# li-guihai/slam-dynamic

Measured on AMD Instinct MI355X. Metric: tracking frames/sec (extract+match+dynamic-cull), KITTI 1241x376, higher is better.
Workload: dtype u8+f32; 1 GPU; KITTI stereo 1241x376 colour pairs, 2000 feat/image: YOLOv3 (640x480, f32 as the reference's cv::dnn, synthetic weights) on the left image -> boxes -> TrackStereo = cvtColor + 2x ORB extract + stereo match + boxTrack + firstSeparate + TrackHomo (SearchByProjection vs the queued frame > 0.2 s back, H/F fit) + Separate + UpdateFrame + SearchByProjection vs the last frame (BASELINE configs[2]); spec ; lanes_per_gpu=256, images_per_frame=2, detector_arithmetic=f32 operands, f32 accumulation (v_mfma_f32_32x32x2_f32), max_detector_boxes_in_a_frame=29

## Files before the change

slam-dynamic_amd/csrc/k_yolo32.h:

```cpp
#pragma once
#include "k_yolo.h"

typedef float sd_f4 __attribute__((ext_vector_type(4)));

struct SdConvArgsF {
    const float* in; const float* wgt; const float* bias; const float* res; float* out;
    const float* zero;
    int N, H, W, cin, cinStride;
    int Ho, Wo, cout, outStride, resStride;
    int ksize, stride, pad, leaky;
    int pair;
    int tilesX, tilesY, groupY;
};

template <int BK, int WM, int MT, int NW>
__global__ void __launch_bounds__(64 * NW, NW == 8 ? 1 : (WM == 2 && BK == 16 ? 3 : 2)) k_conv_f32(SdConvArgsF A)
{
    constexpr int NT = 64 * NW;
    constexpr int WN = NW / WM, BM = 32 * MT * WM, BN = 64 * WN;
    constexpr int LD = BK + 4;
    constexpr int CPR = BK / 4;
    constexpr int XC = (BN * CPR + NT - 1) / NT;
    constexpr int WC = (BM * CPR + NT - 1) / NT;
    constexpr int STAGE = (BM + BN) * LD;
    constexpr int NCH = BK / 8;
    extern __shared__ __align__(16) float smemf[];
    const int tid = threadIdx.x, lane = tid & 63, wv = tid >> 6, r32 = lane & 31, h = lane >> 5;
    const int wm = wv % WM, wn = wv / WM;
    const int perXcd = (A.tilesX + 7) >> 3;
    const int slot = blockIdx.x >> 3, perGroup = perXcd * A.groupY;
    const int grp = slot / perGroup, r = slot - grp * perGroup;
    const int tx = (blockIdx.x & 7) * perXcd + r / A.groupY, ty = grp * A.groupY + r % A.groupY;
    if (tx >= A.tilesX) return;
    const int pix0 = tx * BN, co0 = ty * BM;
    const int npix = A.N * A.Ho * A.Wo;
    int pyi[XC], pxi[XC];
    size_t pbase[XC];
    bool pok[XC];
#pragma unroll
    for (int i = 0; i < XC; i++) {
        const int chunk = tid + NT * i;
        const int p = pix0 + chunk / CPR;
        pok[i] = chunk < BN * CPR && p < npix;
        const int pp = pok[i] ? p : 0;
        const int n = pp / (A.Ho * A.Wo), r = pp - n * (A.Ho * A.Wo);
        const int yo = r / A.Wo, xo = r - yo * A.Wo;
        pyi[i] = yo * A.stride - A.pad; pxi[i] = xo * A.stride - A.pad;
        pbase[i] = (size_t)n * A.H * A.W;
    }
    const int taps = A.ksize * A.ksize;
    const bool pair = BK == 8 && A.pair;
    const int ksteps = pair ? (taps + 1) / 2 : taps * (A.cin / BK);
    const int wrow = pair ? 8 * ksteps : taps * A.cin;
    sd_f16v acc[MT][2];
#pragma unroll
    for (int m = 0; m < MT; m++)
#pragma unroll
        for (int n = 0; n < 2; n++)
#pragma unroll
            for (int r = 0; r < 16; r++) acc[m][n][r] = 0.f;
    constexpr bool DEEP = !(WM == 1 && MT == 2);
    constexpr int NSET = DEEP ? 2 : 1;
    sd_f4 xr[NSET][XC], wr[NSET][WC];
    const float* wptr[WC];
    const float* xptr[XC];
    int winc[WC], xinc[XC];
#pragma unroll
    for (int i = 0; i < WC; i++) {
        const int chunk = tid + NT * i;
        const bool on = chunk < BM * CPR;
        wptr[i] = on ? A.wgt + (size_t)(co0 + chunk / CPR) * wrow + 4 * (chunk % CPR) : A.zero;
        winc[i] = on ? BK : 0;
    }
    int c0 = 0, kh = 0, kw = 0, ps = 0;
    auto retap = [&]() {
#pragma unroll
        for (int i = 0; i < XC; i++) {
            const int chunk = tid + NT * i;
            int dy = kh, dx = kw, coff = 4 * (chunk % CPR);
            bool tapok = true;
            if (BK == 8 && pair) {
                const int tap = 2 * ps + (chunk % CPR);
                dy = tap / A.ksize; dx = tap - dy * A.ksize; coff = 0;
                tapok = tap < taps;
            }
            const int yi = pyi[i] + dy, xi = pxi[i] + dx;
            const bool ok = pok[i] && tapok && yi >= 0 && yi < A.H && xi >= 0 && xi < A.W;
            const float* p = A.in + ((ptrdiff_t)pbase[i] + (ptrdiff_t)yi * A.W + xi) * A.cinStride + coff;
            xptr[i] = ok ? p : A.zero;
            xinc[i] = ok && !pair ? BK : 0;
        }
    };
    retap();
    auto fetch = [&](const int set) {
#pragma unroll
        for (int i = 0; i < WC; i++) { wr[set][i] = *(const sd_f4*)wptr[i]; wptr[i] += winc[i]; }
#pragma unroll
        for (int i = 0; i < XC; i++) { xr[set][i] = *(const sd_f4*)xptr[i]; xptr[i] += xinc[i]; }
        if (BK == 8 && pair) { ps++; retap(); return; }
        c0 += BK;
        if (c0 == A.cin) { c0 = 0; kw++; if (kw == A.ksize) { kw = 0; kh++; } retap(); }
    };
    auto store = [&](int buf, const int set) {
        float* sW = smemf + buf * STAGE;
        float* sX = sW + BM * LD;
#pragma unroll
        for (int i = 0; i < WC; i++) { const int chunk = tid + NT * i; if ((WC * NT == BM * CPR) || chunk < BM * CPR) *(sd_f4*)(sW + (chunk / CPR) * LD + 4 * (chunk % CPR)) = wr[set][i]; }
#pragma unroll
        for (int i = 0; i < XC; i++) { const int chunk = tid + NT * i; if ((XC * NT == BN * CPR) || chunk < BN * CPR) *(sd_f4*)(sX + (chunk / CPR) * LD + 4 * (chunk % CPR)) = xr[set][i]; }
    };
    const int aoff = (32 * MT * wm + r32) * LD + 4 * h, boff = BM * LD + (64 * wn + r32) * LD + 4 * h;
    sd_f4 fa[2][MT], fb[2][2];
    auto frags = [&](int buf, int kc, int slot) {
        const float* base = smemf + buf * STAGE;
#pragma unroll
        for (int m = 0; m < MT; m++) fa[slot][m] = *(const sd_f4*)(base + aoff + 32 * m * LD + 8 * kc);
#pragma unroll
        for (int n = 0; n < 2; n++) fb[slot][n] = *(const sd_f4*)(base + boff + 32 * n * LD + 8 * kc);
    };
    auto mfmas = [&](int slot) {
#pragma unroll
        for (int j = 0; j < 4; j++)
#pragma unroll
            for (int m = 0; m < MT; m++)
#pragma unroll
                for (int n = 0; n < 2; n++)
                    acc[m][n] = __builtin_amdgcn_mfma_f32_32x32x2f32(fa[slot][m][j], fb[slot][n][j], acc[m][n], 0, 0, 0);
    };
    const int myslot = NW == 8 ? (NCH >= 4 ? 2 * (wv >> 2) : (NCH == 2 ? (wv >> 2) : 0)) : 0;
    float* const sBias = smemf + 2 * STAGE;
    sd_f4 bq = sd_f4{0.f, 0.f, 0.f, 0.f};
    if (tid < BM / 4 && co0 + 4 * tid < A.cout) bq = *(const sd_f4*)(A.bias + co0 + 4 * tid);
    fetch(0);
    store(0, 0);
    if (tid < BM / 4) *(sd_f4*)(sBias + 4 * tid) = bq;
    if (ksteps > 1) fetch(NSET - 1);
    if (DEEP && ksteps > 2) fetch(0);
    __syncthreads();
    auto step = [&](const int ks, const int par) {
        const int cur = par;
        frags(cur, 0, 0);
#pragma unroll
        for (int kc = 0; kc < NCH; kc++) {
            if (kc + 1 < NCH) frags(cur, kc + 1, (kc + 1) & 1);
            mfmas(kc & 1);
            if (kc == myslot) {
                if (ks + 1 < ksteps) store(cur ^ 1, DEEP ? par ^ 1 : 0);
                if (ks + 1 + NSET < ksteps) fetch(DEEP ? par ^ 1 : 0);
            }
        }
        __builtin_amdgcn_sched_barrier(0);
        __syncthreads();
        __builtin_amdgcn_sched_barrier(0);
    };
    int ks = 0;
    for (; ks + 1 < ksteps; ks += 2) { step(ks, 0); step(ks + 1, 1); }
    if (ks < ksteps) step(ks, 0);
    if constexpr (WM == 1) {
        constexpr int TWD = 32 * MT, TLD = TWD + 4;
        constexpr int PPI = 64 / (TWD / 4);
        static_assert(NW * 32 * TLD <= 2 * STAGE, "the transpose tiles of the epilogue must fit the staging buffers");
        float* T = smemf + wv * 32 * TLD;
        const int piece = lane % (TWD / 4), prow = lane / (TWD / 4);
        const int cob = co0 + TWD * wm + 4 * piece;
        const sd_f4 bias4 = *(const sd_f4*)(sBias + TWD * wm + 4 * piece);
        __syncthreads();
        auto tail = [&](const bool res, const bool inside) {
            sd_f4 rr[2][32 / PPI];
            if (res) {
#pragma unroll
                for (int n = 0; n < 2; n++)
#pragma unroll
                    for (int it = 0; it < 32 / PPI; it++) {
                        const int p = pix0 + 64 * wn + 32 * n + PPI * it + prow;
                        rr[n][it] = sd_f4{0.f, 0.f, 0.f, 0.f};
                        if (inside || (p < npix && cob < A.cout)) rr[n][it] = *(const sd_f4*)(A.res + (size_t)p * A.resStride + cob);
                    }
                __builtin_amdgcn_s_waitcnt(0x0F70);
            }
#pragma unroll
            for (int n = 0; n < 2; n++) {
#pragma unroll
                for (int m = 0; m < MT; m++)
#pragma unroll
                    for (int g = 0; g < 4; g++)
                        *(sd_f4*)(T + r32 * TLD + 32 * m + 8 * g + 4 * h) = sd_f4{acc[m][n][4 * g], acc[m][n][4 * g + 1], acc[m][n][4 * g + 2], acc[m][n][4 * g + 3]};
                __builtin_amdgcn_fence(__ATOMIC_RELEASE, "wavefront"); __builtin_amdgcn_wave_barrier(); __builtin_amdgcn_fence(__ATOMIC_ACQUIRE, "wavefront");
                const int pb = pix0 + 64 * wn + 32 * n;
#pragma unroll
                for (int it = 0; it < 32 / PPI; it++) {
                    const int pl = PPI * it + prow, p = pb + pl;
                    if (!inside && (p >= npix || cob >= A.cout)) continue;
                    const sd_f4 a = *(const sd_f4*)(T + pl * TLD + 4 * piece);
                    sd_f4 v;
#pragma unroll
                    for (int e = 0; e < 4; e++) {
                        float x = a[e] + bias4[e];
                        if (A.leaky) x = x > 0.f ? x : 0.1f * x;
                        v[e] = x + (res ? rr[n][it][e] : 0.f);
                    }
                    float* dst = A.out + (size_t)p * A.outStride + cob;
                    if (inside || cob + 3 < A.cout) *(sd_f4*)dst = v;
                    else for (int e = 0; e < 4 && cob + e < A.cout; e++) dst[e] = v[e];
                }
                __builtin_amdgcn_fence(__ATOMIC_RELEASE, "wavefront"); __builtin_amdgcn_wave_barrier(); __builtin_amdgcn_fence(__ATOMIC_ACQUIRE, "wavefront");
            }
        };
        const bool inside = pix0 + BN <= npix && co0 + BM <= A.cout;
        if (A.res) { if (inside) tail(true, true); else tail(true, false); }
        else { if (inside) tail(false, true); else tail(false, false); }
    } else {
        auto tail = [&](const bool res, const bool inside) {
            sd_f4 rr[2][MT][4];
            if (res) {
#pragma unroll
                for (int n = 0; n < 2; n++) {
                    const int p = pix0 + 64 * wn + 32 * n + r32;
#pragma unroll
                    for (int m = 0; m < MT; m++)
#pragma unroll
                        for (int g = 0; g < 4; g++) {
                            const int co = co0 + 32 * MT * wm + 32 * m + 8 * g + 4 * h;
                            rr[n][m][g] = sd_f4{0.f, 0.f, 0.f, 0.f};
                            if (inside || (p < npix && co < A.cout)) rr[n][m][g] = *(const sd_f4*)(A.res + (size_t)p * A.resStride + co);
                        }
                }
                __builtin_amdgcn_s_waitcnt(0x0F70);
            }
#pragma unroll
            for (int n = 0; n < 2; n++) {
                const int p = pix0 + 64 * wn + 32 * n + r32;
                if (!inside && p >= npix) continue;
#pragma unroll
                for (int m = 0; m < MT; m++)
#pragma unroll
                    for (int g = 0; g < 4; g++) {
                        const int cl = 32 * MT * wm + 32 * m + 8 * g + 4 * h, co = co0 + cl;
                        if (!inside && co >= A.cout) continue;
                        const sd_f4 b4 = *(const sd_f4*)(sBias + cl);
                        sd_f4 v;
#pragma unroll
                        for (int e = 0; e < 4; e++) {
                            float x = acc[m][n][4 * g + e] + b4[e];
                            if (A.leaky) x = x > 0.f ? x : 0.1f * x;
                            v[e] = x + (res ? rr[n][m][g][e] : 0.f);
                        }
                        float* dst = A.out + (size_t)p * A.outStride + co;
                        if (inside || co + 3 < A.cout) *(sd_f4*)dst = v;
                        else for (int e = 0; e < 4 && co + e < A.cout; e++) dst[e] = v[e];
                    }
            }
        };
        const bool inside = pix0 + BN <= npix && co0 + BM <= A.cout;
        if (A.res) { if (inside) tail(true, true); else tail(true, false); }
        else { if (inside) tail(false, true); else tail(false, false); }
    }
}
#define SD_F32_LDS(BK, WM, MT, NW) (2 * (32 * (MT) * (WM) + 64 * ((NW) / (WM))) * ((BK) + 4) * 4 + 32 * (MT) * (WM) * 4)

__global__ void __launch_bounds__(256) k_blob_from_image_f32(const uint8_t* __restrict__ src, int sw, int sh, size_t sstride, size_t spitch,
                                                             const short4* __restrict__ ct, const short4* __restrict__ rt,
                                                             float* __restrict__ dst, int dw, int dh, int swapRB)
{
    const int img = blockIdx.z;
    const int x = blockIdx.x * 64 + threadIdx.x, y = blockIdx.y * 4 + threadIdx.y;
    if (x >= dw || y >= dh) return;
    const short4 ce = ct[x], re = rt[y];
    const int sx = ce.x, sx1 = min(sx + 1, sw - 1);
    const int r0 = min(max((int)re.x, 0), sh - 1), r1 = min(max((int)re.x + 1, 0), sh - 1);
    const uint8_t* S0 = src + (size_t)img * spitch + (size_t)r0 * sstride;
    const uint8_t* S1 = src + (size_t)img * spitch + (size_t)r1 * sstride;
    uint32_t a0, a1, b0, b1;
    if (sx1 == sx + 1) {
        typedef uint32_t __attribute__((aligned(1))) u32u; typedef uint16_t __attribute__((aligned(1))) u16u;
        a0 = *(const u32u*)(S0 + 3 * sx); b0 = *(const u16u*)(S0 + 3 * sx + 4);
        a1 = *(const u32u*)(S1 + 3 * sx); b1 = *(const u16u*)(S1 + 3 * sx + 4);
    } else {
        a0 = (uint32_t)S0[3 * sx] | ((uint32_t)S0[3 * sx + 1] << 8) | ((uint32_t)S0[3 * sx + 2] << 16) | ((uint32_t)S0[3 * sx1] << 24);
        b0 = (uint32_t)S0[3 * sx1 + 1] | ((uint32_t)S0[3 * sx1 + 2] << 8);
        a1 = (uint32_t)S1[3 * sx] | ((uint32_t)S1[3 * sx + 1] << 8) | ((uint32_t)S1[3 * sx + 2] << 16) | ((uint32_t)S1[3 * sx1] << 24);
        b1 = (uint32_t)S1[3 * sx1 + 1] | ((uint32_t)S1[3 * sx1 + 2] << 8);
    }
    const int p0[6] = {(int)(a0 & 255), (int)((a0 >> 8) & 255), (int)((a0 >> 16) & 255), (int)(a0 >> 24), (int)(b0 & 255), (int)((b0 >> 8) & 255)};
    const int p1[6] = {(int)(a1 & 255), (int)((a1 >> 8) & 255), (int)((a1 >> 16) & 255), (int)(a1 >> 24), (int)(b1 & 255), (int)((b1 >> 8) & 255)};
    float ch[3];
#pragma unroll
    for (int c = 0; c < 3; c++) {
        const int h0 = p0[c] * ce.y + p0[3 + c] * ce.z;
        const int h1 = p1[c] * ce.y + p1[3 + c] * ce.z;
        const int v = ((((int)re.y * (h0 >> 4)) >> 16) + (((int)re.z * (h1 >> 4)) >> 16) + 2) >> 2;
        ch[c] = (float)(v & 255) * (float)(1 / 255.0);
    }
    float* o = dst + ((size_t)img * dh * dw + (size_t)y * dw + x) * 4;
    *(sd_f4*)o = sd_f4{swapRB ? ch[2] : ch[0], ch[1], swapRB ? ch[0] : ch[2], 0.f};
}


__global__ void __launch_bounds__(256) k_upsample_into_f32(const float* __restrict__ a, int C1, int aStride, int h, int w, float* __restrict__ out, int Ct, int N)
{
    const int q = C1 / 4, H2 = 2 * h, W2 = 2 * w;
    const size_t total = (size_t)N * H2 * W2 * q;
    for (size_t i = (size_t)blockIdx.x * 256 + threadIdx.x; i < total; i += (size_t)gridDim.x * 256) {
        const int c4 = (int)(i % q);
        const size_t p = i / q;
        const int x = (int)(p % W2);
        const size_t r = p / W2;
        const int y = (int)(r % H2), n = (int)(r / H2);
        *(sd_f4*)(out + p * Ct + 4 * c4) = *(const sd_f4*)(a + (((size_t)n * h + (y >> 1)) * w + (x >> 1)) * aStride + 4 * c4);
    }
}
```

slam-dynamic_amd/csrc/sd_yolo_api.hip:

```cpp
#include <hip/hip_runtime.h>
#include <cstdio>
#include <cstdlib>
#include <cstring>
#include <cstddef>
#include <cmath>
#include <string>
#include <memory>
#include <vector>
#include "sd_common.h"
#include "sd_yolo.h"

template <typename T>
static void yolo_decode(const sd_yolo* y, const sd_yolo_layer& l, const sd_yolo::Rt& r, int n, float conf_threshold, int rowBase, hipStream_t s)
{
    const float* an = y->anchors;
    const int rows = n * r.H * r.W * 3;
    hipLaunchKernelGGL(HIP_KERNEL_NAME(k_region_decode<T>), dim3((rows + 255) / 256), dim3(256), 0, s, r.as<const T>(), r.outC, r.H, r.W, n, an[2 * l.mask[0]],
                       an[2 * l.mask[0] + 1], an[2 * l.mask[1]], an[2 * l.mask[1] + 1], an[2 * l.mask[2]], an[2 * l.mask[2] + 1],
                       y->netW, y->netH, conf_threshold, rowBase, y->d_dets, y->d_ndet, y->detCap, n == 1 ? y->d_raw : nullptr);
}

extern "C" {

int sd_yolo_v3_layers(sd_yolo_layer* layers, int cap, int* n, float anchors[18])
{
    if (!n) return SD_ERR_INVALID;
    std::vector<sd_yolo_layer> L;
    yolo_v3_layers(L);
    *n = (int)L.size();
    if (anchors) memcpy(anchors, kYoloV3Anchors, sizeof(kYoloV3Anchors));
    if (layers) {
        if (cap < (int)L.size()) return set_err(SD_ERR_CAPACITY, "layer buffer too small");
        memcpy(layers, L.data(), L.size() * sizeof(sd_yolo_layer));
    }
    return SD_OK;
}

static const void* const kYoloKernelFn[SD_YK_COUNT] = {
#define X(id, block, ...) (const void*)__VA_ARGS__,
    SD_YOLO_KERNELS(X)
#undef X
};

static int yolo_kernel_lds(int k, int width)
{
    switch (k) {
    case SD_YK_GLDS_8_1: case SD_YK_GLDS_8_3: return 3 * (512 * 64 + SD_G3_WBYTES);
    case SD_YK_GLDS_4_1: case SD_YK_GLDS_4_3: return 3 * (256 * 64 + SD_G3_WBYTES);
    case SD_YK_G3_80: return SD_G3_LDS(80);
    case SD_YK_G3_160: return SD_G3_LDS(160);
    case SD_YK_F32_8_1_1_8: return SD_F32_LDS(8, 1, 1, 8);
    case SD_YK_F32_16_1_1_4: return SD_F32_LDS(16, 1, 1, 4);
    case SD_YK_F32_16_1_2_4: return SD_F32_LDS(16, 1, 2, 4);
    case SD_YK_F32_16_2_2_4: return SD_F32_LDS(16, 2, 2, 4);
    case SD_YK_WINO_16_2: return SD_WINO_LDS(16, 2);
    case SD_YK_B3_1: return SD_B3_LDS(1);
    case SD_YK_B3_2: return SD_B3_LDS(2);
    case SD_YK_B3F_3: case SD_YK_B3F_4: case SD_YK_B3F_5: case SD_YK_B3F_8: return SD_B3F_LDS(width, 128);
    case SD_YK_B3C_5: case SD_YK_B3C_6: return SD_B3C_LDS(width);
    default: return 0;
    }
}

static int yolo_launch(const SdYoloLaunch& K, void** args, hipStream_t s)
{
    (void)hipLaunchKernel(kYoloKernelFn[K.kernel], dim3(K.gridX, K.gridY), dim3(K.block), args, (size_t)yolo_kernel_lds(K.kernel, K.width), s);
    LAUNCH_CHECK(kYoloKernelInfo[K.kernel].name);
    return SD_OK;
}

static int yolo_raise_lds_limits(const sd_yolo* y)
{
    for (int k = y->f32 ? SD_YK_F32_FIRST : 0; k < (y->f32 ? SD_YK_COUNT : SD_YK_F32_FIRST); k++)
        HIPCHK(sd_raise_lds_limit(kYoloKernelFn[k], yolo_kernel_lds(k, k >= SD_YK_B3C_5 ? SD_B3C_MAXW : SD_B3F_MAXW)));
    HIPCHK(sd_raise_lds_limit((const void*)k_yolo_nms, SD_NMS_LDS));
    return SD_OK;
}

int sd_yolo_create(sd_yolo** out, const sd_yolo_layer* layers, int n_layers, const float anchors[18], int classes, int net_w,
                   int net_h, int max_batch)
{
    return sd_yolo_create_prec(out, layers, n_layers, anchors, classes, net_w, net_h, max_batch, SD_YOLO_F16);
}

int sd_yolo_create_prec(sd_yolo** out, const sd_yolo_layer* layers, int n_layers, const float anchors[18], int classes, int net_w,
                        int net_h, int max_batch, int precision)
{
// ... 286 lines not shown
int sd_yolo_mfma_flops(const sd_yolo* y, double* flops_per_image)
{
    if (!y || !flops_per_image) return SD_ERR_INVALID;
    *flops_per_image = y->mfmaFlops;
    return SD_OK;
}

int sd_yolo_forward_device(sd_yolo* y, const uint8_t* d_bgr, int width, int height, size_t stride, size_t image_pitch, int n,
                           float conf_threshold, void* stream_)
{
    if (!y || !d_bgr || width < 2 || height < 2 || n < 1 || n > y->maxBatch || width > 8192 || height > 8192) return set_err(SD_ERR_INVALID, "bad forward arguments");
    if (!y->weightsLoaded) return set_err(SD_ERR_STATE, "detector weights not loaded");
    hipStream_t s = stream_ ? (hipStream_t)stream_ : y->stream;
    if (y->tabW != width || y->tabH != height) {
        std::vector<int16_t> ct, rt;
        yolo_resize_tables(width, height, y->netW, y->netH, ct, rt);
        HIPCHK(hipMemcpy(y->d_ct, ct.data(), ct.size() * 2, hipMemcpyHostToDevice));
        HIPCHK(hipMemcpy(y->d_rt, rt.data(), rt.size() * 2, hipMemcpyHostToDevice));
        y->tabW = width; y->tabH = height;
    }
    const bool f32 = y->f32, ov = y->overlap;
    hipStream_t sb = ov ? y->sPre : s, sd = ov ? y->sPost : s;
    if (ov && y->haveL0) HIPCHK(hipStreamWaitEvent(sb, y->evL0, 0));
    {
        dim3 blk(64, 4), grd((y->netW + 63) / 64, (y->netH + 3) / 4, n);
        if (f32) hipLaunchKernelGGL(k_blob_from_image_f32, grd, blk, 0, sb, d_bgr, width, height, stride, image_pitch, y->d_ct, y->d_rt, y->d_blob8, y->netW, y->netH, 1);
        else hipLaunchKernelGGL(k_blob_from_image, grd, blk, 0, sb, d_bgr, width, height, stride, image_pitch, y->d_ct, y->d_rt, y->d_blob4, y->netW, y->netH, 1);
    }
    LAUNCH_CHECK(f32 ? "k_blob_from_image_f32" : "k_blob_from_image");
    if (ov) {
        HIPCHK(hipEventRecord(y->evBlob, sb));
        HIPCHK(hipStreamWaitEvent(s, y->evBlob, 0));
    }
    bool cleared = !f32;
    if (cleared) HIPCHK(hipMemsetAsync(y->d_ndet, 0, (size_t)n * 4, s));
    int head = 0;
    bool headGuard = ov && y->haveDecoded;
    const void* cur = f32 ? (const void*)y->d_blob8.get() : (const void*)y->d_blob4.get();
    int H = y->netH, W = y->netW, Cs = f32 ? 4 : 32;
    int rowBase = 0;
    for (size_t i = 0; i < y->L.size(); i++) {
        const sd_yolo_layer& l = y->L[i];
        const sd_yolo::Rt& r = y->R[i];
        if (l.type == SD_YOLO_CONV) {
            if (headGuard && i + 1 < y->L.size() && y->L[i + 1].type == SD_YOLO_YOLO) { HIPCHK(hipStreamWaitEvent(s, y->evDecoded, 0)); headGuard = false; }
            const SdYoloLaunch K = yolo_plan_launch(l, r, i == 0, n);
            const void* bias = y->d_bias + r.bOff;
            const void* res = nullptr; int resStride = 0;
            if (i + 1 < y->L.size() && y->L[i + 1].type == SD_YOLO_SHORTCUT && y->R[i + 1].alias) {
                const sd_yolo::Rt& rf = y->R[yolo_resolve((int)i + 1, y->L[i + 1].from[0])];
                res = rf.out; resStride = rf.outC;
            }
            int rc;
            if (K.kernel == SD_YK_CONV_FIRST) {
                const _Float16* blob = y->d_blob4; const _Float16* wgt = y->d_wgt + r.wOff; _Float16* out = r.as<_Float16>();
                int Ho = r.H, Wo = r.W, cout = l.filters, outStride = r.outC, leaky = l.leaky;
                void* args[] = {&blob, &wgt, &bias, &out, &n, &Ho, &Wo, &cout, &outStride, &leaky};
                rc = yolo_launch(K, args, s);
            } else if (r.cls == SD_YC_F16) {
                SdConvArgs A;
                A.zero = y->d_zero; A.in = (const _Float16*)cur; A.wgt = y->d_wgt + r.wOff; A.bias = (const float*)bias; A.res = (const _Float16*)res; A.out = r.as<_Float16>();
                A.N = n; A.H = H; A.W = W; A.cin = r.cinPad; A.cinStride = Cs;
                A.Ho = r.H; A.Wo = r.W; A.cout = l.filters; A.coutPad = r.coutPad; A.outStride = r.outC; A.outOff = 0; A.resStride = resStride;
                A.ksize = l.size; A.stride = l.stride; A.pad = l.size / 2; A.leaky = l.leaky;
                void* args[] = {&A};
                rc = yolo_launch(K, args, s);
            } else if (r.cls == SD_YC_WINO) {
                SdWinoArgs A;
                A.V = y->d_V; A.U = y->d_wgtW + r.wOffW; A.bias = (const float*)bias; A.res = (const float*)res; A.out = r.as<float>(); A.zero = (const float*)y->d_zero.get();
                A.N = n; A.H = r.H; A.W = r.W; A.th = (r.H + 1) / 2; A.tw = (r.W + 1) / 2;
                A.cin = r.cinPad; A.cout = l.filters; A.outStride = r.outC; A.resStride = resStride; A.leaky = l.leaky;
                A.tilesX = K.tilesX; A.tilesY = K.tilesY; A.groupY = K.groupY;
                hipLaunchKernelGGL(k_wino_input, dim3(K.inputGrid), dim3(256), 0, s, (const float*)cur, n, H, W, r.cinPad, Cs, A.th, A.tw, y->d_V);
                LAUNCH_CHECK("k_wino_input");
                void* args[] = {&A};
                rc = yolo_launch(K, args, s);
            } else {
                SdConvArgsF A;
                A.in = (const float*)cur; A.wgt = y->d_wgt32 + r.wOff; A.bias = (const float*)bias; A.res = (const float*)res; A.out = r.as<float>(); A.zero = (const float*)y->d_zero.get();
                A.N = n; A.H = H; A.W = W; A.cin = i == 0 ? 8 : r.cinPad; A.cinStride = Cs; A.pair = i == 0 ? 1 : 0;
                A.Ho = r.H; A.Wo = r.W; A.cout = l.filters; A.outStride = r.outC; A.resStride = resStride;
                A.ksize = l.size; A.stride = l.stride; A.pad = l.size / 2; A.leaky = l.leaky;
                A.tilesX = K.tilesX; A.tilesY = K.tilesY; A.groupY = K.groupY;
                const uint4* wq = y->d_wgtB + r.wOffB;
                void* args[] = {&A, &wq};
                rc = yolo_launch(K, args, s);
            }
            if (rc != SD_OK) return rc;
        } else if (l.type == SD_YOLO_SHORTCUT) {
            if (!r.alias) return set_err(SD_ERR_UNSUPPORTED, "unfused [shortcut] is not implemented");
        } else if (l.type == SD_YOLO_ROUTE && l.nfrom == 2) {
            const int fa = yolo_resolve((int)i, l.from[0]), fb = yolo_resolve((int)i, l.from[1]);
            const int src = yolo_resolve(fa, -1);
            const sd_yolo::Rt& ra = y->R[src]; const sd_yolo::Rt& rb = y->R[fb];
            if (f32 && r.alias) {
                const size_t quads = (size_t)n * r.H * r.W * (ra.C / 4);
                hipLaunchKernelGGL(k_upsample_into_f32, dim3((unsigned)std::min<size_t>((quads + 255) / 256, 4096)), dim3(256), 0, s, ra.as<const float>(), ra.C, ra.outC, ra.H, ra.W,
                                   r.as<float>(), r.C, n);
                LAUNCH_CHECK("k_upsample_into_f32");
            } else {
                const int hc = f32 ? 2 : 1, piece = 8 / hc;
                if (ra.outC != ra.C || rb.outC != rb.C || (ra.C % piece) || (rb.C % piece))
                    return set_err(SD_ERR_UNSUPPORTED, f32 ? "route inputs must be dense, channels % 4 == 0" : "route inputs must be dense, channels % 8 == 0");
                hipLaunchKernelGGL(k_upsample_concat, dim3(2048), dim3(256), 0, s, ra.as<const _Float16>(), hc * ra.C, ra.H, ra.W, rb.as<const _Float16>(), hc * rb.C,
                                   r.as<_Float16>(), n);
                LAUNCH_CHECK("k_upsample_concat");
            }
        } else if (l.type == SD_YOLO_YOLO) {
            if (ov && head < 3) {
                HIPCHK(hipEventRecord(y->evHead[head], s));
                HIPCHK(hipStreamWaitEvent(sd, y->evHead[head], 0));
                if (head == 0 && y->haveNms) HIPCHK(hipStreamWaitEvent(sd, y->evNms, 0));
            }
            if (!cleared) { HIPCHK(hipMemsetAsync(y->d_ndet, 0, (size_t)n * 4, sd)); cleared = true; }
            if (f32) yolo_decode<float>(y, l, r, n, conf_threshold, rowBase, sd);
            else yolo_decode<_Float16>(y, l, r, n, conf_threshold, rowBase, sd);
            LAUNCH_CHECK("k_region_decode");
            rowBase += r.H * r.W * 3;
            head++;
        }
        if (ov && i == 0) { HIPCHK(hipEventRecord(y->evL0, s)); y->haveL0 = true; }
        if (l.type != SD_YOLO_YOLO && l.type != SD_YOLO_UPSAMPLE) { cur = r.out; H = r.H; W = r.W; Cs = r.outC; }
        if (l.type == SD_YOLO_YOLO) { cur = r.out; }
    }
    if (!cleared) HIPCHK(hipMemsetAsync(y->d_ndet, 0, (size_t)n * 4, sd));
    if (ov) { HIPCHK(hipEventRecord(y->evDecoded, sd)); y->haveDecoded = true; }
    y->lastN = n;
    if (!stream_) { HIPCHK(hipStreamSynchronize(s)); if (ov) HIPCHK(hipStreamSynchronize(y->sPost)); }
    return SD_OK;
}

int sd_yolo_download_layer(sd_yolo* y, int layer, int image, uint16_t* out)
{
    if (!y || !out || layer < 0 || layer >= (int)y->L.size() || image < 0 || image >= y->lastN) return SD_ERR_INVALID;
    const sd_yolo::Rt& r = y->R[layer];
    if (!r.out) return set_err(SD_ERR_INVALID, "layer has no materialised output");
    HIPCHK(hipDeviceSynchronize());
    const size_t pix = (size_t)r.H * r.W, eb = y->f32 ? 4 : 2;
    const unsigned char* src = r.as<const unsigned char>() + (size_t)image * pix * r.outC * eb;
    if (r.outC == r.C) {
        HIPCHK(hipMemcpy(out, src, pix * r.C * eb, hipMemcpyDeviceToHost));
    } else {
        HIPCHK(hipMemcpy2D(out, (size_t)r.C * eb, src, (size_t)r.outC * eb, (size_t)r.C * eb, pix, hipMemcpyDeviceToHost));
    }
    return SD_OK;
}

int sd_yolo_precision(const sd_yolo* y, int* precision)
{
    if (!y || !precision) return SD_ERR_INVALID;
    *precision = y->b3 ? SD_YOLO_F32X3 : (y->wino ? SD_YOLO_F32W : (y->f32 ? SD_YOLO_F32 : SD_YOLO_F16));
    return SD_OK;
}

int sd_yolo_download_region(sd_yolo* y, float* rows, int* total_rows)
{
    if (!y || !rows || y->lastN != 1) return set_err(SD_ERR_STATE, "region rows are kept only after a forward with n == 1");
    HIPCHK(hipDeviceSynchronize());
    HIPCHK(hipMemcpy(rows, y->d_raw, (size_t)y->totalRows * (5 + y->classes) * 4, hipMemcpyDeviceToHost));
    if (total_rows) *total_rows = y->totalRows;
    return SD_OK;
}

static int yolo_nms(sd_yolo* y, int image, int frame_cols, int frame_rows, float conf_threshold, float nms_threshold,
                    std::vector<SdDet>& d, std::vector<YRect>& rects, std::vector<int>& kept)
{
    HIPCHK(hipDeviceSynchronize());
// ... 148 lines not shown
```

slam-dynamic_amd/csrc/sd_yolo_plan.h:

```cpp
#pragma once
#include <algorithm>
#include <cstddef>
#include <vector>
#include "sd_frontend.h"

#define SD_CV_BM 64
#define SD_CV_BN 256
#define SD_C3_BM 128
#define SD_C3_BN 256
#define SD_C3_BK 32
#define SD_C3_MAXW 80
#define SD_G3_BM 128
#define SD_G3_BN 512
#define SD_B3F_MAXW 160
#define SD_B3C_MAXW 80
#define SD_F32_GRID(tx, ty) (unsigned)((((tx) + 7) / 8) * 8 * (ty))

static const float kYoloV3Anchors[18] = {10, 13, 16, 30, 33, 23, 30, 61, 62, 45, 59, 119, 116, 90, 156, 198, 373, 326};

static inline void yolo_v3_layers(std::vector<sd_yolo_layer>& L)
{
    auto conv = [&](int filters, int size, int stride, int bn = 1, int leaky = 1) {
        sd_yolo_layer l = {}; l.type = SD_YOLO_CONV; l.filters = filters; l.size = size; l.stride = stride; l.batch_normalize = bn; l.leaky = leaky;
        L.push_back(l);
// ... 91 lines not shown
                r.wOffB = P.wTotalB; P.wTotalB += (size_t)(r.coutPad / 128) * (l.size * l.size * (r.cinPad / 16)) * 2 * 6 * 64;
                P.mfmaFlopsBf16 += 6 * flops;
            } else P.mfmaFlops += flops;
            P.nconv++;
        } else if (l.type == SD_YOLO_SHORTCUT) {
            const int f = yolo_resolve(i, l.from[0]);
            if (f < 0 || f >= i || P.R[f].H != H || P.R[f].W != W || P.R[f].C != C) return {SD_ERR_INVALID, "bad shortcut"};
            r.H = H; r.W = W; r.C = C; r.outC = C;
        } else if (l.type == SD_YOLO_ROUTE) {
            const int f0 = yolo_resolve(i, l.from[0]);
            if (f0 < 0 || f0 >= i) return {SD_ERR_INVALID, "bad route"};
            r.H = P.R[f0].H; r.W = P.R[f0].W; r.C = P.R[f0].C;
            if (l.nfrom == 2) {
                const int f1 = yolo_resolve(i, l.from[1]);
                if (f1 < 0 || f1 >= i || P.R[f1].H != r.H || P.R[f1].W != r.W) return {SD_ERR_INVALID, "bad route"};
                r.C += P.R[f1].C;
            }
            r.outC = r.C;
        } else if (l.type == SD_YOLO_UPSAMPLE) {
            r.H = 2 * H; r.W = 2 * W; r.C = C; r.outC = C;
        } else if (l.type == SD_YOLO_YOLO) {
            if (C != 3 * (5 + classes)) return {SD_ERR_INVALID, "[yolo] input must have 3*(5+classes) channels"};
            r.H = H; r.W = W; r.C = C; r.outC = C;
            P.totalRows += H * W * 3;
        } else return {SD_ERR_INVALID, "unknown layer type"};
        H = r.H; W = r.W; C = r.C;
        if ((l.type == SD_YOLO_CONV) && (r.C % 4) && r.C != 3 * (5 + classes)) return {SD_ERR_UNSUPPORTED, "filters must be a multiple of 4"};
    }
    return {SD_OK, nullptr};
}

#define SD_YOLO_KERNELS(X) \
    X(CONV_FIRST, 256, k_conv_first) \
    X(GLDS_8_1, 512, k_conv_glds<8, 1>) \
    X(GLDS_4_1, 256, k_conv_glds<4, 1>) \
    X(GLDS_8_3, 512, k_conv_glds<8, 3>) \
    X(GLDS_4_3, 256, k_conv_glds<4, 3>) \
    X(G3_80, 512, k_conv3x3_glds<80>) \
    X(G3_160, 512, k_conv3x3_glds<160>) \
    X(C3_FLAT, 256, k_conv3x3_flat) \
    X(MFMA_64, 256, k_conv_mfma<64>) \
    X(MFMA_32, 256, k_conv_mfma<32>) \
    X(F32_8_1_1_8, 512, k_conv_f32<8, 1, 1, 8>) \
    X(F32_16_1_1_4, 256, k_conv_f32<16, 1, 1, 4>) \
    X(F32_16_1_2_4, 256, k_conv_f32<16, 1, 2, 4>) \
    X(F32_16_2_2_4, 256, k_conv_f32<16, 2, 2, 4>) \
    X(WINO_16_2, 256, k_wino_gemm_f32<16, 2>) \
    X(B3_1, 256, k_conv_b3<1>) \
    X(B3_2, 256, k_conv_b3<2>) \
    X(B3F_3, 256, k_conv3x3_b3<3, 2, 2>) \
    X(B3F_4, 256, k_conv3x3_b3<4, 2, 2>) \
    X(B3F_5, 256, k_conv3x3_b3<5, 2, 2>) \
    X(B3F_8, 256, k_conv3x3_b3<8, 2, 2>) \
    X(B3C_5, 512, k_conv3x3_b3c<5>) \
    X(B3C_6, 512, k_conv3x3_b3c<6>)
enum SdYoloKernel {
#define X(id, block, ...) SD_YK_##id,
    SD_YOLO_KERNELS(X)
#undef X
    SD_YK_COUNT, SD_YK_F32_FIRST = SD_YK_F32_8_1_1_8
};
static const struct { const char* name; int block; } kYoloKernelInfo[SD_YK_COUNT] = {
#define X(id, block, ...) {#__VA_ARGS__, block},
    SD_YOLO_KERNELS(X)
#undef X
};

struct SdYoloLaunch {
    int kernel = 0;
    unsigned gridX = 1, gridY = 1;
    int block = 0;
    int tilesX = 0, tilesY = 0, groupY = 0;
    int width = 0;
    unsigned inputGrid = 0;
};

static inline int f32_group_y(int tilesY, int bm, int kdim)
{
    int g = 1;
    while (2 * g <= tilesY && tilesY % (2 * g) == 0 && (size_t)(2 * g) * bm * kdim * 4 <= (size_t)2560 * 1024) g *= 2;
    return g;
}

static inline SdYoloLaunch yolo_plan_launch(const sd_yolo_layer& l, const SdYoloLayerPlan& r, bool first, int n)
{
    SdYoloLaunch K;
    const int npix = n * r.H * r.W, taps = l.size * l.size;
    const bool s3 = l.size == 3 && l.stride == 1;
    auto tiles = [&](SdYoloKernel k, int bn, int tilesY, int groupY) {
        K.kernel = k; K.tilesX = (npix + bn - 1) / bn; K.tilesY = tilesY; K.groupY = groupY; K.gridX = SD_F32_GRID(K.tilesX, K.tilesY);
    };
    auto grid2 = [&](SdYoloKernel k, int bn, int gridY) { K.kernel = k; K.gridX = (npix + bn - 1) / bn; K.gridY = gridY; };
    switch (r.cls) {
    case SD_YC_F16: {
        const bool flat3 = s3 && r.W <= 160 && l.filters % SD_G3_BM == 0 && r.cinPad % 32 == 0 && npix >= SD_G3_BN;
        if (first) { K.kernel = SD_YK_CONV_FIRST; K.gridX = (unsigned)(((size_t)n * r.H * r.W + 255) / 256); }
        else if (!flat3 && r.cinPad % 32 == 0 && npix >= 512 && (l.size == 1 || l.filters >= SD_G3_BM / 2)) {
            const int ct = r.coutPad / SD_G3_BM;
            const bool big = ((npix + 511) / 512) * ct >= 256;
            if (l.size == 1) grid2(big ? SD_YK_GLDS_8_1 : SD_YK_GLDS_4_1, big ? 512 : 256, ct);
            else grid2(big ? SD_YK_GLDS_8_3 : SD_YK_GLDS_4_3, big ? 512 : 256, ct);
        } else if (flat3) grid2(r.W <= 80 ? SD_YK_G3_80 : SD_YK_G3_160, SD_G3_BN, l.filters / SD_G3_BM);
        else if (s3 && r.W <= SD_C3_MAXW && l.filters % SD_C3_BM == 0 && r.cinPad % SD_C3_BK == 0) grid2(SD_YK_C3_FLAT, SD_C3_BN, l.filters / SD_C3_BM);
        else grid2(r.cinPad % 64 == 0 ? SD_YK_MFMA_64 : SD_YK_MFMA_32, SD_CV_BN, (l.filters + SD_CV_BM - 1) / SD_CV_BM);
        break;
    }
    case SD_YC_F32: {
        const int kdim = (first ? 8 : r.cinPad) * taps;
        if (first) tiles(SD_YK_F32_8_1_1_8, 512, (l.filters + 31) / 32, f32_group_y((l.filters + 31) / 32, 32, kdim));
        else if (l.filters <= 32) tiles(SD_YK_F32_16_1_1_4, 256, 1, 1);
        else if (l.filters <= 64) tiles(SD_YK_F32_16_1_2_4, 256, 1, 1);
        else tiles(SD_YK_F32_16_2_2_4, 128, r.coutPad / 128, f32_group_y(r.coutPad / 128, 128, kdim));
        break;
    }
    case SD_YC_WINO: {
        const size_t nblk = (size_t)n * ((r.H + 1) / 2) * ((r.W + 1) / 2);
        K.kernel = SD_YK_WINO_16_2; K.tilesX = (int)((nblk + 63) / 64); K.tilesY = r.coutPad / 128; K.groupY = K.tilesY;
        K.gridX = SD_F32_GRID(K.tilesX, K.tilesY);
        K.inputGrid = (unsigned)std::min<size_t>((nblk * (r.cinPad / 4) + 255) / 256, 65536);
        break;
    }
    case SD_YC_B3: tiles(SD_YK_B3_2, 128, r.coutPad / 128, f32_group_y(r.coutPad / 128, 128, r.cinPad * taps * 3 / 2)); break;
    case SD_YC_B3_64: tiles(SD_YK_B3_1, 256, 1, 1); break;
    case SD_YC_B3_FLAT: {
        const int np = (4 * (128 + 2 * r.W + 2) + 255) / 256;
        tiles(np <= 3 ? SD_YK_B3F_3 : np == 4 ? SD_YK_B3F_4 : np == 5 ? SD_YK_B3F_5 : SD_YK_B3F_8, 128, r.coutPad / 128, f32_group_y(r.coutPad / 128, 128, r.cinPad * taps * 3 / 2));
        K.width = r.W;
        break;
    }
    case SD_YC_B3_FLATC: {
        const int np = (4 * (512 + 2 * r.W + 2) + 511) / 512;
        tiles(np <= 5 ? SD_YK_B3C_5 : SD_YK_B3C_6, 512, r.coutPad / 64, f32_group_y(r.coutPad / 64, 64, r.cinPad * 9 * 3 / 2));
        K.gridX = 8 * (unsigned)std::min(((K.tilesX + 7) / 8) * K.tilesY, 32);
        K.width = r.W;
        break;
    }
    default: break;
    }
    K.block = kYoloKernelInfo[K.kernel].block;
    return K;
}
```

Before: 1085 frames/s.

## Precompute magic divisors and tap masks to cut f32 conv address arithmetic

Result: faster. 1099 frames/s, median of 6 (+1.3%).

```diff
diff --git a/slam-dynamic_amd/csrc/k_yolo32.h b/slam-dynamic_amd/csrc/k_yolo32.h
--- a/slam-dynamic_amd/csrc/k_yolo32.h
+++ b/slam-dynamic_amd/csrc/k_yolo32.h
@@ -11,7 +11,21 @@
     int ksize, stride, pad, leaky;
     int pair;
     int tilesX, tilesY, groupY;
+    unsigned mHoWo, sHoWo, mWo, sWo;
+    unsigned mPerGroup, sPerGroup, mGroupY, sGroupY;
+    int tapCol, tapRow;
 };
+
+__device__ __forceinline__ unsigned sd_udiv(unsigned n, unsigned m, unsigned s) { return (__umulhi(n, m) + n) >> s; }
+
+typedef float sd_f2 __attribute__((ext_vector_type(2)));
+__device__ __forceinline__ sd_f4 sd_f32_tail(const sd_f4 a, const sd_f4 b, const float slope, const sd_f4 r, const bool res)
+{
+    sd_f2 x0 = a.xy + b.xy, x1 = a.zw + b.zw;
+    x0 = __builtin_elementwise_max(x0, x0 * slope); x1 = __builtin_elementwise_max(x1, x1 * slope);
+    if (res) { x0 += r.xy; x1 += r.zw; }
+    return sd_f4{x0.x, x0.y, x1.x, x1.y};
+}
 
 template <int BK, int WM, int MT, int NW>
 __global__ void __launch_bounds__(64 * NW, NW == 8 ? 1 : (WM == 2 && BK == 16 ? 3 : 2)) k_conv_f32(SdConvArgsF A)
@@ -27,31 +41,24 @@
     extern __shared__ __align__(16) float smemf[];
     const int tid = threadIdx.x, lane = tid & 63, wv = tid >> 6, r32 = lane & 31, h = lane >> 5;
     const int wm = wv % WM, wn = wv / WM;
-    const int perXcd = (A.tilesX + 7) >> 3;
-    const int slot = blockIdx.x >> 3, perGroup = perXcd * A.groupY;
-    const int grp = slot / perGroup, r = slot - grp * perGroup;
-    const int tx = (blockIdx.x & 7) * perXcd + r / A.groupY, ty = grp * A.groupY + r % A.groupY;
-    if (tx >= A.tilesX) return;
+    const float* const in = A.in; const float* const wgt = A.wgt; const float* const zero = A.zero;
+    const int H = A.H, W = A.W, cin = A.cin, cinStride = A.cinStride, Ho = A.Ho, Wo = A.Wo, ksize = A.ksize, stride = A.stride, pad = A.pad;
+    const int tilesX = A.tilesX, groupY = A.groupY;
+    const int N = A.N, HoWo = Ho * Wo, npix = N * HoWo;
+    const unsigned mHoWo = A.mHoWo, sHoWo = A.sHoWo, mWo = A.mWo, sWo = A.sWo;
+    const ptrdiff_t tapCol = A.tapCol, tapRow = A.tapRow;
+    const float slope = A.leaky ? 0.1f : 1.f;
+    const int perXcd = (tilesX + 7) >> 3;
+    const unsigned slot = blockIdx.x >> 3, perGroup = perXcd * groupY;
+    const unsigned grp = sd_udiv(slot, A.mPerGroup, A.sPerGroup), r = slot - grp * perGroup, rq = sd_udiv(r, A.mGroupY, A.sGroupY);
+    const int tx = (blockIdx.x & 7) * perXcd + rq, ty = grp * groupY + (r - rq * groupY);
+    if (tx >= tilesX) return;
     const int pix0 = tx * BN, co0 = ty * BM;
-    const int npix = A.N * A.Ho * A.Wo;
-    int pyi[XC], pxi[XC];
-    size_t pbase[XC];
-    bool pok[XC];
-#pragma unroll
-    for (int i = 0; i < XC; i++) {
-        const int chunk = tid + NT * i;
-        const int p = pix0 + chunk / CPR;
-        pok[i] = chunk < BN * CPR && p < npix;
-        const int pp = pok[i] ? p : 0;
-        const int n = pp / (A.Ho * A.Wo), r = pp - n * (A.Ho * A.Wo);
-        const int yo = r / A.Wo, xo = r - yo * A.Wo;
-        pyi[i] = yo * A.stride - A.pad; pxi[i] = xo * A.stride - A.pad;
-        pbase[i] = (size_t)n * A.H * A.W;
-    }
-    const int taps = A.ksize * A.ksize;
-    const bool pair = BK == 8 && A.pair;
-    const int ksteps = pair ? (taps + 1) / 2 : taps * (A.cin / BK);
-    const int wrow = pair ? 8 * ksteps : taps * A.cin;
+    const int taps = ksize * ksize;
+    constexpr bool pair = BK == 8;
+    __builtin_assume(pair || cin >= 2 * BK);
+    const int ksteps = pair ? (taps + 1) / 2 : taps * (cin / BK);
+    const int wrow = pair ? 8 * ksteps : taps * cin;
     sd_f16v acc[MT][2];
 #pragma unroll
     for (int m = 0; m < MT; m++)
@@ -61,45 +68,87 @@
             for (int r = 0; r < 16; r++) acc[m][n][r] = 0.f;
     constexpr bool DEEP = !(WM == 1 && MT == 2);
     constexpr int NSET = DEEP ? 2 : 1;
+    static_assert(XC * NT == BN * CPR && NT % CPR == 0, "every thread stages XC activation chunks, all of them the same piece of their rows");
     sd_f4 xr[NSET][XC], wr[NSET][WC];
     const float* wptr[WC];
     const float* xptr[XC];
+    const char* xtrue[XC];
+    unsigned tapmask[XC];
     int winc[WC], xinc[XC];
-#pragma unroll
-    for (int i = 0; i < WC; i++) {
-        const int chunk = tid + NT * i;
-        const bool on = chunk < BM * CPR;
-        wptr[i] = on ? A.wgt + (size_t)(co0 + chunk / CPR) * wrow + 4 * (chunk % CPR) : A.zero;
-        winc[i] = on ? BK : 0;
-    }
-    int c0 = 0, kh = 0, kw = 0, ps = 0;
+    const int q = tid % CPR;
+    {
+        constexpr unsigned D = NT / CPR;
+        const unsigned dn = sd_udiv(D, mHoWo, sHoWo), dr = D - dn * HoWo, dy = sd_udiv(dr, mWo, sWo), dx = dr - dy * Wo;
+        const unsigned p = pix0 + tid / CPR;
+        unsigned n = sd_udiv(p, mHoWo, sHoWo);
+        const unsigned pr = p - n * HoWo;
+        unsigned yo = sd_udiv(pr, mWo, sWo), xo = pr - yo * Wo;
+        const unsigned rowrep = ksize == 1 ? 1u : 1u | 1u << ksize | 1u << 2 * ksize;
+        const unsigned rowlow = (1u << ksize) - 1u;
+#pragma unroll
+        for (int i = 0; i < XC; i++) {
+            if (i > 0) {
+                xo += dx; const bool cx = xo >= (unsigned)Wo; xo -= cx ? Wo : 0;
+                yo += dy + (cx ? 1 : 0); const bool cy = yo >= (unsigned)Ho; yo -= cy ? Ho : 0;
+                n += dn + (cy ? 1 : 0);
+            }
+            const int yi = __mul24((int)yo, stride) - pad, xi = __mul24((int)xo, stride) - pad;
+            const int lx = max(-xi, 0), hx = min(W - xi, ksize), ly = max(-yi, 0), hy = min(H - yi, ksize);
+            const unsigned mk = __umul24((1u << hx) - 1u - lx, rowrep) & ((1u << __umul24(hy, ksize)) - (1u + __umul24(ly, rowlow)));
+            tapmask[i] = n < (unsigned)N ? (pair ? mk >> q : mk) : 0;
+            const int pixel = __mul24((int)__umul24(n, H) + yi, W) + xi;
+            xtrue[i] = (const char*)in + ((long long)pixel * (4 * cinStride) + (pair ? 4 * cinStride : 16) * q);
+        }
+    }
+    {
+        constexpr int DW = NT / CPR;
+        const char* const w0 = (const char*)(wgt + (size_t)co0 * (unsigned)wrow) + (__umul24(tid / CPR, wrow) * 4u + 16u * q);
+#pragma unroll
+        for (int i = 0; i < WC; i++) {
+            const bool on = (WC * NT == BM * CPR) || tid + NT * i < BM * CPR;
+            wptr[i] = on ? (const float*)(w0 + (size_t)(4 * DW * i) * (unsigned)wrow) : zero;
+            winc[i] = on ? BK : 0;
+        }
+    }
+    int c0 = 0, kw = 0, pdx = q;
+    unsigned tapbit = 1;
+    auto select = [&]() {
+#pragma unroll
+        for (int i = 0; i < XC; i++) {
+            const bool ok = (tapmask[i] & tapbit) != 0;
+            xptr[i] = ok ? (const float*)xtrue[i] : zero;
+            xinc[i] = ok && !pair ? BK : 0;
+        }
+    };
     auto retap = [&]() {
-#pragma unroll
-        for (int i = 0; i < XC; i++) {
-            const int chunk = tid + NT * i;
-            int dy = kh, dx = kw, coff = 4 * (chunk % CPR);
-            bool tapok = true;
-            if (BK == 8 && pair) {
-                const int tap = 2 * ps + (chunk % CPR);
-                dy = tap / A.ksize; dx = tap - dy * A.ksize; coff = 0;
-                tapok = tap < taps;
-            }
-            const int yi = pyi[i] + dy, xi = pxi[i] + dx;
-            const bool ok = pok[i] && tapok && yi >= 0 && yi < A.H && xi >= 0 && xi < A.W;
-            const float* p = A.in + ((ptrdiff_t)pbase[i] + (ptrdiff_t)yi * A.W + xi) * A.cinStride + coff;
-            xptr[i] = ok ? p : A.zero;
-            xinc[i] = ok && !pair ? BK : 0;
-        }
-    };
-    retap();
+        if (pair) {
+            pdx += 2;
+            const bool wrap = pdx >= ksize;
+            pdx -= wrap ? ksize : 0;
+            const ptrdiff_t d = wrap ? tapRow + tapCol : 2 * tapCol;
+#pragma unroll
+            for (int i = 0; i < XC; i++) xtrue[i] += d;
+            tapbit <<= 2;
+        } else {
+            kw++;
+            const bool wrap = kw == ksize;
+            if (wrap) kw = 0;
+            const ptrdiff_t d = wrap ? tapRow : tapCol;
+#pragma unroll
+            for (int i = 0; i < XC; i++) xtrue[i] += d;
+            tapbit <<= 1;
+        }
+        select();
+    };
+    select();
     auto fetch = [&](const int set) {
 #pragma unroll
         for (int i = 0; i < WC; i++) { wr[set][i] = *(const sd_f4*)wptr[i]; wptr[i] += winc[i]; }
 #pragma unroll
         for (int i = 0; i < XC; i++) { xr[set][i] = *(const sd_f4*)xptr[i]; xptr[i] += xinc[i]; }
-        if (BK == 8 && pair) { ps++; retap(); return; }
+        if (pair) { retap(); return; }
         c0 += BK;
-        if (c0 == A.cin) { c0 = 0; kw++; if (kw == A.ksize) { kw = 0; kh++; } retap(); }
+        if (c0 == cin) { c0 = 0; retap(); }
     };
     auto store = [&](int buf, const int set) {
         float* sW = smemf + buf * STAGE;
@@ -129,8 +178,7 @@
     };
     const int myslot = NW == 8 ? (NCH >= 4 ? 2 * (wv >> 2) : (NCH == 2 ? (wv >> 2) : 0)) : 0;
     float* const sBias = smemf + 2 * STAGE;
-    sd_f4 bq = sd_f4{0.f, 0.f, 0.f, 0.f};
-    if (tid < BM / 4 && co0 + 4 * tid < A.cout) bq = *(const sd_f4*)(A.bias + co0 + 4 * tid);
+    const sd_f4 bq = *(const sd_f4*)(A.bias + co0 + 4 * (tid % (BM / 4)));
     fetch(0);
     store(0, 0);
     if (tid < BM / 4) *(sd_f4*)(sBias + 4 * tid) = bq;
@@ -192,13 +240,7 @@
                     const int pl = PPI * it + prow, p = pb + pl;
                     if (!inside && (p >= npix || cob >= A.cout)) continue;
                     const sd_f4 a = *(const sd_f4*)(T + pl * TLD + 4 * piece);
-                    sd_f4 v;
-#pragma unroll
-                    for (int e = 0; e < 4; e++) {
-                        float x = a[e] + bias4[e];
-                        if (A.leaky) x = x > 0.f ? x : 0.1f * x;
-                        v[e] = x + (res ? rr[n][it][e] : 0.f);
-                    }
+                    const sd_f4 v = sd_f32_tail(a, bias4, slope, rr[n][it], res);
                     float* dst = A.out + (size_t)p * A.outStride + cob;
                     if (inside || cob + 3 < A.cout) *(sd_f4*)dst = v;
                     else for (int e = 0; e < 4 && cob + e < A.cout; e++) dst[e] = v[e];
@@ -238,13 +280,7 @@
                         const int cl = 32 * MT * wm + 32 * m + 8 * g + 4 * h, co = co0 + cl;
                         if (!inside && co >= A.cout) continue;
                         const sd_f4 b4 = *(const sd_f4*)(sBias + cl);
-                        sd_f4 v;
-#pragma unroll
-                        for (int e = 0; e < 4; e++) {
-                            float x = acc[m][n][4 * g + e] + b4[e];
-                            if (A.leaky) x = x > 0.f ? x : 0.1f * x;
-                            v[e] = x + (res ? rr[n][m][g][e] : 0.f);
-                        }
+                        const sd_f4 v = sd_f32_tail(sd_f4{acc[m][n][4 * g], acc[m][n][4 * g + 1], acc[m][n][4 * g + 2], acc[m][n][4 * g + 3]}, b4, slope, rr[n][m][g], res);
                         float* dst = A.out + (size_t)p * A.outStride + co;
                         if (inside || co + 3 < A.cout) *(sd_f4*)dst = v;
                         else for (int e = 0; e < 4 && co + e < A.cout; e++) dst[e] = v[e];
diff --git a/slam-dynamic_amd/csrc/sd_yolo_api.hip b/slam-dynamic_amd/csrc/sd_yolo_api.hip
--- a/slam-dynamic_amd/csrc/sd_yolo_api.hip
+++ b/slam-dynamic_amd/csrc/sd_yolo_api.hip
@@ -3,6 +3,7 @@
 #include <cstdlib>
 #include <cstring>
 #include <cstddef>
+#include <climits>
 #include <cmath>
 #include <string>
 #include <memory>
@@ -455,7 +456,13 @@
                 A.Ho = r.H; A.Wo = r.W; A.cout = l.filters; A.outStride = r.outC; A.resStride = resStride;
                 A.ksize = l.size; A.stride = l.stride; A.pad = l.size / 2; A.leaky = l.leaky;
                 A.tilesX = K.tilesX; A.tilesY = K.tilesY; A.groupY = K.groupY;
-                const uint4* wq = y->d_wgtB + r.wOffB;
+                const SdF32Setup S = yolo_f32_setup(K.tilesX, K.groupY, r.H, r.W, W, l.size, Cs);
+                if (S.tapRow > INT_MAX || S.tapRow < INT_MIN || (long long)n * r.H * r.W + 512 > INT_MAX || (long long)n * H * W > INT_MAX || (long long)n * H >= (1 << 23) || W >= (1 << 23))
+                    return set_err(SD_ERR_UNSUPPORTED, "convolution too large for the f32 kernels' 32-bit pixel index");
+                A.mHoWo = S.hoWo.m; A.sHoWo = S.hoWo.s; A.mWo = S.wo.m; A.sWo = S.wo.s;
+                A.mPerGroup = S.perGroup.m; A.sPerGroup = S.perGroup.s; A.mGroupY = S.groupY.m; A.sGroupY = S.groupY.s;
+                A.tapCol = (int)S.tapCol; A.tapRow = (int)S.tapRow;
+                const uint4* wq =y->d_wgtB + r.wOffB;
                 void* args[] = {&A, &wq};
                 rc = yolo_launch(K, args, s);
             }
diff --git a/slam-dynamic_amd/csrc/sd_yolo_plan.h b/slam-dynamic_amd/csrc/sd_yolo_plan.h
--- a/slam-dynamic_amd/csrc/sd_yolo_plan.h
+++ b/slam-dynamic_amd/csrc/sd_yolo_plan.h
@@ -197,6 +197,25 @@
     return g;
 }
 
+struct SdMagic { unsigned m, s; };
+static inline SdMagic sd_magic_div(unsigned d)
+{
+    unsigned s = 0;
+    while ((1ull << s) < d) s++;
+    return {(unsigned)((((1ull << (32 + s)) + d - 1) / d) - (1ull << 32)), s};
+}
+static inline unsigned sd_magic_quot(unsigned n, SdMagic k) { return ((unsigned)(((unsigned long long)n * k.m) >> 32) + n) >> k.s; }
+
+struct SdF32Setup { SdMagic hoWo, wo, perGroup, groupY; long long tapCol, tapRow; };
+static inline SdF32Setup yolo_f32_setup(int tilesX, int groupY, int Ho, int Wo, int W, int ksize, int cinStride)
+{
+    SdF32Setup S;
+    S.hoWo = sd_magic_div((unsigned)(Ho * Wo)); S.wo = sd_magic_div((unsigned)Wo);
+    S.perGroup = sd_magic_div((unsigned)(((tilesX + 7) / 8) * groupY)); S.groupY = sd_magic_div((unsigned)groupY);
+    S.tapCol = 4ll * cinStride; S.tapRow = 4ll * (W - ksize + 1) * cinStride;
+    return S;
+}
+
 static inline SdYoloLaunch yolo_plan_launch(const sd_yolo_layer& l, const SdYoloLayerPlan& r, bool first, int n)
 {
     SdYoloLaunch K;
```
